# cs2mosa/Heterogeneous-MOE-for-Diffusion-models

Hardware: AMD Instinct MI355X
Metric: denoise-steps/sec (fwd+bwd) on 4x32x32 latents (higher is better)
Workload: dtype bf16

## Files before the change

### heterogeneous-moe-for-diffusion-models_amd/csrc/bwd6.hip

```cpp
#include "common.h"
#include "conv_args.h"
#include "conv6_common.h"
#include "hdmoe.h"
#include "conv6_body.h"
#include "conv7_body.h"
#include "wgrad6_body.h"
#include "wgrad7_body.h"
#include "wgrad8_body.h"
#include "conv6s_body.h"

namespace {

template <int MT, int NT, int TWS, int OT>
__global__ __launch_bounds__(512) void bwd6_kernel(C6Args c, W6Args a3, W6Args a5, int G6, int ibs, int obs) {
  const int b = blockIdx.x;
  if (b < G6) { conv6_body<MT, NT>(c, b, G6); return; }
  int r = b - G6;
  const int bx = r % ibs; r /= ibs;
  const int by = r % obs;
  const int z = r / obs;
  if (z < a3.chunks) wgrad6_body<3, TWS, OT, false>(a3, bx, by, z);
  else wgrad6_body<5, TWS, OT, false>(a5, bx, by, z - a3.chunks);
}

template <int MT, int NT, int TWS, int OT>
void launch_bwd6(const C6Plan& cp, const W6DualPlan& wp, hipStream_t stream) {
  static unsigned long long attr = 0;
  if (hdmoe_first_on_device(attr)) { (void)hipFuncSetAttribute((const void*)bwd6_kernel<MT, NT, TWS, OT>, hipFuncAttributeMaxDynamicSharedMemorySize, 160 * 1024); }
  const size_t lds = cp.lds > wp.lds ? cp.lds : wp.lds;
  const unsigned grid = cp.G + (unsigned)(wp.ibs * wp.obs * (wp.c[0].chunks + wp.c[1].chunks));
  hipLaunchKernelGGL((bwd6_kernel<MT, NT, TWS, OT>), dim3(grid), dim3(512), lds, stream, cp.a, wp.c[0], wp.c[1], (int)cp.G, wp.ibs, wp.obs);
}

template <int CO, int KMASK, int TWS, int OT, int EPI = 0>
__global__ __launch_bounds__(512) void bwd7_kernel(C7Args c, W6Args a3, W6Args a5, int G7, int ibs, int obs) {
  const int b = blockIdx.x;
  if (b < G7) { conv7_body<CO, KMASK, TWS == 4, EPI>(c, b, G7); return; }
  int r = b - G7;
  if (TWS == 5 && OT == 0) {
    const int nbx3 = a3.Cin / (32 * a3.icw), nby3 = a3.Cout / (32 * a3.ocw), n3 = nbx3 * nby3 * a3.chunks;
    if (r < n3) {
      const int bx = r % nbx3; r /= nbx3;
      const int by = r % nby3, z = r / nby3, pairs = a3.icw * a3.ocw;
      if (pairs == 0) wgrad7_body<3>(a3, bx, by, z);
      else if (pairs == 4) wgrad8_body3<4, 8>(a3, bx, by, z);
      else if (pairs == 2) wgrad8_body3<2, 8>(a3, bx, by, z);
      else wgrad8_body3<2, 16>(a3, bx, by, z);
      return;
    }
    r -= n3;
    const int bx = r % ibs; r /= ibs;
    wgrad7_body<5>(a5, bx, r % obs, r / obs);
  } else if (OT > 0) {
    const int bx = r % ibs; r /= ibs;
    const int by = r % obs;
    const int z = r / obs;
    if (z < a3.chunks) wgrad6_body<3, TWS, OT == 0 ? 1 : OT, false>(a3, bx, by, z);
    else wgrad6_body<5, TWS, OT == 0 ? 1 : OT, false>(a5, bx, by, z - a3.chunks);
  }
}

template <int CO, int KMASK, int TWS, int OT, int EPI = 0>
void launch_bwd7(const C7Plan& cp, const W6DualPlan& wp, hipStream_t stream) {
  static unsigned long long attr = 0;
  if (hdmoe_first_on_device(attr)) { (void)hipFuncSetAttribute((const void*)bwd7_kernel<CO, KMASK, TWS, OT, EPI>, hipFuncAttributeMaxDynamicSharedMemorySize, 160 * 1024); }
  const size_t clds = cp.lds + (EPI ? C7Lds<TWS == 4>::film_extra(CO) : 0);
  const size_t lds = clds > wp.lds ? clds : wp.lds;
  const int obs = OT == 0 ? wp.c[0].Cout / 32 : wp.obs;
  unsigned nw = (unsigned)(wp.ibs * obs * (wp.c[0].chunks + wp.c[1].chunks));
  if (OT == 0) nw = (unsigned)((wp.c[0].Cin / (32 * wp.c[0].icw)) * (wp.c[0].Cout / (32 * wp.c[0].ocw)) * wp.c[0].chunks + wp.ibs * obs * wp.c[1].chunks);
  hipLaunchKernelGGL((bwd7_kernel<CO, KMASK, TWS, OT, EPI>), dim3(cp.G + nw), dim3(512), lds, stream, cp.a, wp.c[0], wp.c[1], (int)cp.G, wp.ibs, obs);
}

template <int NT, int TWS, int OT>
__global__ __launch_bounds__(512) void bwd6s_kernel(C6SArgs c, W6Args a3, int G6, int ibs, int obs) {
  const int b = blockIdx.x;
  if (b < G6) { conv6s_body<NT>(c, b, G6); return; }
  int r = b - G6;
  const int bx = r % ibs; r /= ibs;
  wgrad6_body<3, TWS, OT, true>(a3, bx, r % obs, r / obs);
}
template <int NT, int TWS, int OT>
void launch_bwd6s(const C6SPlan& cp, const W6DualPlan& wp, hipStream_t stream) {
  static unsigned long long attr = 0;
  if (hdmoe_first_on_device(attr)) { (void)hipFuncSetAttribute((const void*)bwd6s_kernel<NT, TWS, OT>, hipFuncAttributeMaxDynamicSharedMemorySize, 160 * 1024); }
  const size_t lds = cp.lds > wp.lds ? cp.lds : wp.lds;
  const unsigned grid = cp.G + (unsigned)(wp.ibs * wp.obs * wp.c[0].chunks);
  hipLaunchKernelGGL((bwd6s_kernel<NT, TWS, OT>), dim3(grid), dim3(512), lds, stream, cp.sa, wp.c[0], (int)cp.G, wp.ibs, wp.obs);
}

}

extern "C" {

int hdmoe_conv_bwd6s(const void* x, const void* dy, const void* wd, void* dx, float* const* G, const int* seg, int ngroups, long wd_stride,
                     long wd_plane, int N, int H, int W, int Cin, int Cout, const int* kh, const int* kw, const int* pt, const int* pl,
                     float alpha, void* ws, long ws_bytes, const float* in_scale, const float* in_shift, int in_relu, int hi_only, hipStream_t stream) {
  if (!dx || !wd || ngroups < 1 || ngroups > HDMOE_MAX_GROUPS || Cout % 16) return 1;
  W6DualPlan wp;
  if (wgrad6_plan_split(x, dy, G, seg, ngroups, N, H, W, Cin, Cout, kh, kw, pt, pl, ws, ws_bytes, wp)) return 1;
  if ((in_scale == nullptr) != (in_shift == nullptr) || (in_scale && (ngroups != 1 || seg))) return HDMOE_EINVAL;
  wp.c[0].in_scale = in_scale; wp.c[0].in_shift = in_shift; wp.c[0].in_relu = in_relu;
  wp.c[0].hi_only = hi_only ? 1 : 0;
  const ConvArgs c = conv_dgrad_args(dy, wd, dx, seg, ngroups, wd_stride, N, H, W, Cin, Cout, kh, kw, pt, pl, alpha);
  C6SPlan cp;
  if (conv6s_plan(c, wd_plane, nullptr, cp)) return 1;
  cp.sa.nprod = hi_only ? 1 : 3;
  hdmoe_count_selection(HDMOE_SEL_BWD6S);
  conv_pick<2, 1>(cp.NT, [&](auto Nt) { conv_pick<5, 4>(wp.TWS, [&](auto Tws) { conv_pick<2, 1>(wp.OT, [&](auto Ot) {
    launch_bwd6s<decltype(Nt)::value, decltype(Tws)::value, decltype(Ot)::value>(cp, wp, stream);
  }); }); });
  return hdmoe_launch_status();
}

int hdmoe_conv_bwd6(const void* x, const void* dy, const void* wd, void* dx, float* const* G, const int* seg, int ngroups, long wd_stride,
                    int N, int H, int W, int Cin, int Cout, const int* kh, const int* kw, const int* pt, const int* pl, float alpha,
                    void* ws, long ws_bytes, int dtype, hipStream_t stream) {
  if (dtype != HDMOE_BF16 || !dx || !wd || ngroups < 1 || ngroups > HDMOE_MAX_GROUPS || Cout % 16) return 1;
  W6DualPlan wp;
  if (wgrad6_plan_dual(x, dy, G, seg, ngroups, N, H, W, Cin, Cout, kh, kw, pt, pl, ws, ws_bytes, dtype, wp)) return 1;
  const ConvArgs c = conv_dgrad_args(dy, wd, dx, seg, ngroups, wd_stride, N, H, W, Cin, Cout, kh, kw, pt, pl, alpha);
  {
    C7Plan cp7;
    if (!conv7_plan(c, dtype, cp7) && cp7.kmask == 3 && (cp7.w16 != 0) == (wp.TWS == 4)) {
      if (wp.TWS == 5) {
        hdmoe_count_selection(HDMOE_SEL_BWD7_32);
        if (wp.c[0].chunks) {
          hdmoe_count_selection(HDMOE_SEL_BWD7_32_WGRAD8);
          hdmoe_count_selection(wp.c[0].icw == 2 ? (wp.c[0].ocw == 2 ? HDMOE_SEL_WGRAD8_C22 : HDMOE_SEL_WGRAD8_C21)
                                                 : (wp.c[0].ocw == 2 ? HDMOE_SEL_WGRAD8_C12 : HDMOE_SEL_WGRAD8_C11));
        }
        if (wp.c[1].chunks) hdmoe_count_selection(HDMOE_SEL_BWD7_32_WGRAD7);
      } else {
        hdmoe_count_selection(wp.OT == 2 ? HDMOE_SEL_BWD7_16_OT2 : HDMOE_SEL_BWD7_16_OT1);
      }
      conv_pick<2, 1>(cp7.CO, [&](auto Co) {
        if (wp.TWS == 5) launch_bwd7<decltype(Co)::value, 3, 5, 0>(cp7, wp, stream);
        else conv_pick<2, 1>(wp.OT, [&](auto Ot) { launch_bwd7<decltype(Co)::value, 3, 4, decltype(Ot)::value>(cp7, wp, stream); });
      });
      return hdmoe_launch_status();
    }
  }
  C6Plan cp;
  if (conv6_plan(c, dtype, cp)) return 1;
  hdmoe_count_selection(HDMOE_SEL_BWD6);
  conv_pick<2, 1>(cp.MT, [&](auto M) { conv_pick<2, 1>(cp.NT, [&](auto Nt) { conv_pick<5, 4>(wp.TWS, [&](auto Tws) { conv_pick<2, 1>(wp.OT, [&](auto Ot) {
    launch_bwd6<decltype(M)::value, decltype(Nt)::value, decltype(Tws)::value, decltype(Ot)::value>(cp, wp, stream);
  }); }); }); });
  return hdmoe_launch_status();
}

int hdmoe_conv_bwd6_film(const void* x, const void* dy, const void* wd, void* dx, float* const* G, const int* seg, int ngroups, long wd_stride,
                         int N, int H, int W, int Cin, int Cout, const int* kh, const int* kw, const int* pt, const int* pl, float alpha,
                         void* ws, long ws_bytes, const void* film_u, const float* film_e, const unsigned char* film_mask, float* film_de,
                         float film_p, int dtype, hipStream_t stream) {
  if (dtype != HDMOE_BF16 || !dx || !wd || ngroups < 1 || ngroups > HDMOE_MAX_GROUPS || Cout % 16) return 1;
  if (!film_u || !film_e || !film_de || ((uintptr_t)film_u & 15) || ((uintptr_t)film_e & 15)) return 1;
  if (film_p < 0.f || film_p >= 1.f || (film_p > 0.f) != (film_mask != nullptr)) return HDMOE_EINVAL;
  W6DualPlan wp;
  if (wgrad6_plan_dual(x, dy, G, seg, ngroups, N, H, W, Cin, Cout, kh, kw, pt, pl, ws, ws_bytes, dtype, wp)) return 1;
  const ConvArgs c = conv_dgrad_args(dy, wd, dx, seg, ngroups, wd_stride, N, H, W, Cin, Cout, kh, kw, pt, pl, alpha);
  C7Plan cp7;
  if (conv7_plan(c, dtype, cp7) || cp7.kmask != 3 || (cp7.w16 != 0) != (wp.TWS == 4)) return 1;
  const bool big = wp.TWS == 5, small = wp.TWS == 4 && cp7.CO == 2 && wp.OT == 2;
  if (!big && !small) return 1;
  cp7.a.film_u = film_u; cp7.a.film_e = film_e; cp7.a.film_mask = film_mask; cp7.a.film_de = film_de;
  cp7.a.film_inv = film_p > 0.f ? 1.f / (1.f - film_p) : 1.f;
  hdmoe_count_selection(HDMOE_SEL_FILM_DGRAD);
  if (big) {
    hdmoe_count_selection(HDMOE_SEL_BWD7_32);
    if (wp.c[0].chunks) {
      hdmoe_count_selection(HDMOE_SEL_BWD7_32_WGRAD8);
      hdmoe_count_selection(wp.c[0].icw == 2 ? (wp.c[0].ocw == 2 ? HDMOE_SEL_WGRAD8_C22 : HDMOE_SEL_WGRAD8_C21)
                                             : (wp.c[0].ocw == 2 ? HDMOE_SEL_WGRAD8_C12 : HDMOE_SEL_WGRAD8_C11));
    }
    if (wp.c[1].chunks) hdmoe_count_selection(HDMOE_SEL_BWD7_32_WGRAD7);
    if (cp7.CO == 2) launch_bwd7<2, 3, 5, 0, 1>(cp7, wp, stream); else launch_bwd7<1, 3, 5, 0, 1>(cp7, wp, stream);
  } else {
    hdmoe_count_selection(HDMOE_SEL_BWD7_16_OT2);
    launch_bwd7<2, 3, 4, 2, 1>(cp7, wp, stream);
  }
  return hdmoe_launch_status();
}

}
```

### heterogeneous-moe-for-diffusion-models_amd/csrc/conv7.hip

```cpp
#include "conv_args.h"
#include "hdmoe.h"
#include "conv7_body.h"

namespace {

template <int CO, int KMASK, bool W16>
__global__ __launch_bounds__(512) void conv7_kernel(C7Args a) { conv7_body<CO, KMASK, W16>(a, blockIdx.x, gridDim.x); }

}

constexpr int C7_MIN_IMAGES = 192;

int conv7_plan(const ConvArgs& c, int dtype, C7Plan& plan) {
  if (dtype != HDMOE_BF16 || c.stride != 1 || c.ones || c.Cphys != c.Cin || c.Ipad != c.Cin || c.Cin % 32 || c.Cin > 256 || c.Cstore != c.Cout) return 1;
  if (c.Cout % 32 || c.Cout > 256) return 1;
  const bool w16 = c.H == 16;
  if (!((c.H == 32 && c.W == 32) || (c.H == 16 && c.W == 16)) || c.Ho != c.H || c.Wo != c.W || c.N < C7_MIN_IMAGES) return 1;
  int kmask = 0;
  long maxtaps = 0;
  for (int g = 0; g < c.ngroups; ++g) {
    const int k = c.kh[g];
    if (c.kw[g] != k || (k != 3 && k != 5 && k != 7) || c.pt[g] != (k - 1) / 2 || c.pl[g] != (k - 1) / 2) return 1;
    kmask |= k == 3 ? 1 : (k == 5 ? 2 : 4);
    if ((long)k * k > maxtaps) maxtaps = (long)k * k;
  }
  const long xbytes = (long)c.N * c.H * c.W * c.Cin * 2;
  const long wbytes = ((long)(c.ngroups - 1) * c.wstride + maxtaps * c.Cout * c.Cin) * 2;
  if (!conv_align_extent_ok({c.x, c.w, c.y, c.res}, {xbytes, wbytes, (long)c.N * c.H * c.W * c.Cout})) return 1;
  C7Args& a = plan.a;
  a.x = c.x; a.w = c.w; a.y = c.y; a.res = c.res; a.seg = c.seg; a.wstride = c.wstride;
  a.N = c.N; a.Cin = c.Cin; a.Cout = c.Cout; a.ngroups = c.ngroups; a.alpha = c.alpha; a.beta = c.beta;
  a.xbytes = (int)xbytes; a.wbytes = (int)wbytes;
  a.dbg = 0;
  a.film_u = nullptr; a.film_e = nullptr; a.film_mask = nullptr; a.film_de = nullptr; a.film_inv = 1.f;
  a.stamps = (unsigned long long*)hdmoe_debug_stamp_buffer();
  for (int g = 0; g < HDMOE_MAX_GROUPS; ++g) a.ks[g] = c.kh[g];
  conv_sort_groups_desc(a.ks, a.order, c.ngroups);
  const long gcap = 256;
  const long units = w16 ? (c.N + 1) / 2 + c.ngroups : c.N;
  plan.G = (unsigned)(units < gcap ? units : gcap);
  plan.CO = c.Cout % 64 == 0 ? 2 : 1;
  plan.w16 = w16 ? 1 : 0;
  plan.lds = w16 ? C7Lds<true>::BYTES : C7Lds<false>::BYTES;
  plan.kmask = (kmask & 4) ? 7 : 3;
  return 0;
}

template <int CO, int KMASK, bool W16>
static void conv7_launch_t(const C7Plan& p, hipStream_t stream) {
  static unsigned long long attr = 0;
  if (hdmoe_first_on_device(attr)) { (void)hipFuncSetAttribute((const void*)conv7_kernel<CO, KMASK, W16>, hipFuncAttributeMaxDynamicSharedMemorySize, C7Lds<W16>::BYTES); }
  hipLaunchKernelGGL((conv7_kernel<CO, KMASK, W16>), dim3(p.G), dim3(512), C7Lds<W16>::BYTES, stream, p.a);
}

void conv7_launch(const C7Plan& p, hipStream_t stream) {
  conv_pick<2, 1>(p.CO, [&](auto Co) { conv_pick<7, 3>(p.kmask, [&](auto Km) { conv_pick<1, 0>(p.w16 != 0, [&](auto W16) {
    conv7_launch_t<decltype(Co)::value, decltype(Km)::value, decltype(W16)::value != 0>(p, stream);
  }); }); });
}

int conv7_try_launch(const ConvArgs& c, int dtype, hipStream_t stream) {
  C7Plan plan;
  if (conv7_plan(c, dtype, plan)) return 1;
  hdmoe_count_selection(plan.w16 ? HDMOE_SEL_CONV7_16 : HDMOE_SEL_CONV7_32);
  conv7_launch(plan, stream);
  return hdmoe_launch_status();
}
```

### heterogeneous-moe-for-diffusion-models_amd/csrc/conv7_body.h

```cpp
#pragma once
#include <type_traits>
#include <utility>
#include "common.h"
#include "conv6_common.h"

namespace {

struct C7Args {
  const void* x; const void* w; void* y; const void* res; const int* seg;
  long wstride;
  int N, Cin, Cout, ngroups;
  int ks[HDMOE_MAX_GROUPS], order[HDMOE_MAX_GROUPS];
  float alpha, beta;
  int xbytes, wbytes;
  int dbg;
  unsigned long long* stamps;
  const void* film_u;
  const float* film_e;
  const unsigned char* film_mask;
  float* film_de;
  float film_inv;
};

template <bool W16> struct C7Geo;
template <> struct C7Geo<false> {
  static constexpr int IMG = 32, MB = 4, ROWB = 35 * 64, TILE = (32 * 35 + 3) * 64, WBUF = 8192, TCO = 4, PPW = 8, HBOFF = 0;
  static constexpr int ZBYTES = 38 * 64;
};
template <> struct C7Geo<true> {
  static constexpr int IMG = 16, MB = 2, ROWB = 19 * 64, TILE = (32 * 19 + 3) * 64, WBUF = 28672, TCO = 14, PPW = 4, HBOFF = 16 * 19 * 64;
  static constexpr int ZBYTES = HBOFF + 22 * 64;
};
template <bool W16> struct C7Lds {
  using GEO = C7Geo<W16>;
  static constexpr int T0 = 2 * GEO::WBUF;
  static constexpr int ZROW = T0 + 2 * GEO::TILE;
  static constexpr int BYTES = ZROW + GEO::ZBYTES;
  static constexpr int film_bytes(int co) { return 8 * (W16 ? 2 : 1) * 32 * co * 4; }
  static constexpr bool film_in_ring(int co) { return BYTES + film_bytes(co) > 160 * 1024; }
  static constexpr int film_extra(int co) { return film_in_ring(co) ? 0 : film_bytes(co); }
};

template <int KS, int CO, int TCO> struct C7Sched {
  static constexpr int T = TCO / CO;
  static constexpr int SPC = (KS + T - 1) / T;
  static constexpr int NS = KS * SPC;
  static constexpr int ky0(int i) { return (KS * i) / SPC; }
  static constexpr int nt(int i) { return (KS * (i + 1)) / SPC - (KS * i) / SPC; }
};

struct C7Unit { int g, n, n2, ks; };

template <typename F, int... I> DEVI void c7_static_for_impl(F&& f, std::integer_sequence<int, I...>) { (f(std::integral_constant<int, I>{}), ...); }
template <int N, typename F> DEVI void c7_static_for(F&& f) { c7_static_for_impl(f, std::make_integer_sequence<int, N>{}); }
template <int N> DEVI void c7_wait_barrier() { asm volatile("s_waitcnt vmcnt(%0) lgkmcnt(0)\n\ts_barrier" :: "n"(N) : "memory"); }

template <int CO, int KMASK, bool W16, int EPI = 0>
DEVI void conv7_body(const C7Args& a, const int bid, const int G) {
#if __HIP_DEVICE_COMPILE__
  using GEO = C7Geo<W16>;
  using L = C7Lds<W16>;
  constexpr int MB = GEO::MB, IMG = GEO::IMG, ROWB = GEO::ROWB, TILE = GEO::TILE, WBUF = GEO::WBUF, TCO = GEO::TCO, PPW = GEO::PPW;
  constexpr int T0 = L::T0, ZROW = L::ZROW;
  constexpr int NSTORE = MB * CO * 2;
  extern __shared__ __attribute__((aligned(1024))) unsigned char lds[];
  const int tid = threadIdx.x, lane = tid & 63;
  const int wave = __builtin_amdgcn_readfirstlane(tid >> 6);
  const int r = lane & 31, h = lane >> 5;
  const __amdgpu_buffer_rsrc_t rx = __builtin_amdgcn_make_buffer_rsrc(const_cast<void*>(a.x), 0, a.xbytes, 0x00020000);
  const __amdgpu_buffer_rsrc_t rw = __builtin_amdgcn_make_buffer_rsrc(const_cast<void*>(a.w), 0, a.wbytes, 0x00020000);
  const int CI = a.Cin >> 5;
  const int cin2 = a.Cin * 2;
  int nstamp = 0;
  auto stamp = [&](int tag) {
    if (a.stamps && bid == 0 && lane == 0 && nstamp < 63) {
      a.stamps[wave * 64 + nstamp] = ((unsigned long long)tag << 56) | (__builtin_amdgcn_s_memtime() & 0x00FFFFFFFFFFFFFFull);
      ++nstamp;
    }
  };
  stamp(1);

  int cum[HDMOE_MAX_GROUPS + 1];
  cum[0] = 0;
#pragma unroll
  for (int i = 0; i < HDMOE_MAX_GROUPS; ++i) {
    int cnt = 0;
    if (i < a.ngroups) { const int g = a.order[i]; cnt = a.seg ? a.seg[g + 1] - a.seg[g] : a.N; }
    cum[i + 1] = cum[i] + (W16 ? (cnt + 1) >> 1 : cnt);
  }
  const int total = cum[HDMOE_MAX_GROUPS];
  auto unit_at = [&](int q, C7Unit& u) -> bool {
    const int pos = q * G + ((q & 1) ? G - 1 - bid : bid);
    if (pos >= total) return false;
    int slot = 0;
#pragma unroll
    for (int i = 1; i < HDMOE_MAX_GROUPS; ++i) slot += (i < a.ngroups && pos >= cum[i]) ? 1 : 0;
    int base = 0, g = 0;
#pragma unroll
    for (int i = 0; i < HDMOE_MAX_GROUPS; ++i) if (i == slot) { base = cum[i]; g = a.order[i]; }
    int ks = 3;
#pragma unroll
    for (int i = 0; i < HDMOE_MAX_GROUPS; ++i) if (i == g) ks = a.ks[i];
    const int s0 = a.seg ? a.seg[g] : 0, s1 = a.seg ? a.seg[g + 1] : a.N;
    u.g = g; u.ks = ks;
    if (W16) { u.n = s0 + 2 * (pos - base); u.n2 = u.n + 1 < s1 ? u.n + 1 : -1; }
    else { u.n = s0 + pos - base; u.n2 = -1; }
    return true;
  };

  for (int i = tid; i < 33 * 12; i += 512) {
    const int off = (i / 12) * ROWB + (i % 12) * 16;
    *reinterpret_cast<uint4*>(lds + T0 + off) = make_uint4(0, 0, 0, 0);
    *reinterpret_cast<uint4*>(lds + T0 + TILE + off) = make_uint4(0, 0, 0, 0);
  }
  for (int i = tid; i < GEO::ZBYTES / 16; i += 512) *reinterpret_cast<uint4*>(lds + ZROW + i * 16) = make_uint4(0, 0, 0, 0);

  const int dpx = lane >> 2;
  const unsigned xlane = (unsigned)(dpx * cin2 + (((lane & 3) ^ (((3 + dpx) >> 2) & 3)) << 4));
  const unsigned wlane = (unsigned)(dpx * cin2 + (((lane & 3) ^ ((dpx >> 2) & 3)) << 4));
  int acol[7];
#pragma unroll
  for (int cc = 0; cc < 7; ++cc) {
    const int col = (W16 ? (r & 15) : r) + cc;
    acol[cc] = (col << 6) + ((h ^ ((col >> 2) & 3)) << 4) + (W16 ? (r >> 4) * GEO::HBOFF : 0);
  }
  const int wl = (r << 6) + ((h ^ ((r >> 2) & 3)) << 4);

  auto issue_tile = [&](const C7Unit& u, int c, int tb) {
    const int lbase = T0 + tb * TILE + 3 * 64;
#pragma unroll
    for (int k = 0; k < PPW; ++k) {
      if (W16) {
        const int img = k >> 1, row = 2 * wave + (k & 1);
        const int n = img ? u.n2 : u.n;
        const int so = (n * 16 + row) * 16 * cin2 + c * 64;
        const unsigned vo = n < 0 ? 0xFFFFFFFFu : xlane;
        __builtin_amdgcn_raw_ptr_buffer_load_lds(rx, (lptr_t)(lds + lbase + (img * 16 + row) * ROWB), 16, vo, n < 0 ? 0 : so, 0, 0);
      } else {
        const int row = 4 * wave + (k >> 1), half = k & 1;
        const int so = ((u.n * 32 + row) * 32 + half * 16) * cin2 + c * 64;
        __builtin_amdgcn_raw_ptr_buffer_load_lds(rx, (lptr_t)(lds + lbase + row * ROWB + half * 1024), 16, xlane, so, 0, 0);
      }
    }
  };
  auto issue_wstage = [&](int g, int ks, int c, int blk, int kx, int ky0, int nt, int sp) {
#pragma unroll
    for (int j = 0; j < (2 * TCO + 7) / 8; ++j) {
      const int pi = wave + 8 * j;
      const int ts = pi / (2 * CO), pc = pi % (2 * CO);
      if (ts < nt) {
        const int tap = (ky0 + ts) * ks + kx;
        const int so = (int)(((long)g * a.wstride + (long)(tap * a.Cout + blk * 32 * CO + pc * 16) * a.Cin) * 2) + c * 64;
        __builtin_amdgcn_raw_ptr_buffer_load_lds(rw, (lptr_t)(lds + sp * WBUF + pi * 1024), 16, wlane, so, 0, 0);
      }
    }
  };

  C7Unit cur, nxt;
  int q = 0;
  if (!unit_at(q, cur)) return;
  bool has_next = unit_at(q + 1, nxt);
  int tp = 0, sp = 0;
  auto nt0_of = [](int ks) { return ks == 3 ? C7Sched<3, CO, GEO::TCO>::nt(0) : (ks == 5 ? C7Sched<5, CO, GEO::TCO>::nt(0) : C7Sched<7, CO, GEO::TCO>::nt(0)); };
  const int nblk = a.Cout / (32 * CO);
  issue_wstage(cur.g, cur.ks, 0, 0, 0, 0, nt0_of(cur.ks), 0);
  issue_tile(cur, 0, 0);
  bool first = true;

  auto run_unit = [&](auto ks_tag) {
    constexpr int KS = decltype(ks_tag)::value;
    using S = C7Sched<KS, CO, TCO>;
    constexpr int P = (KS - 1) / 2, Q = 3 - P;
    for (int blk = 0; blk < nblk; ++blk) {
    const bool last_blk = blk == nblk - 1;
    f32x16 acc[MB][CO];
#pragma unroll
    for (int m = 0; m < MB; ++m)
#pragma unroll
      for (int b = 0; b < CO; ++b) acc[m][b] = (f32x16)(0.f);

    for (int c = 0; c < CI; ++c) {
      const bool last_chunk = c == CI - 1;
      const bool same_tile = last_chunk && !last_blk && CI == 1;
      const bool tile_next = (!last_chunk || (!last_blk && CI > 1) || (last_blk && has_next)) && !((a.dbg & 2) && last_chunk);
      const int tbase = T0 + tp * TILE;
      c7_static_for<S::NS>([&](auto s_c) {
        constexpr int s = decltype(s_c)::value;
        constexpr int kx = s / S::SPC, si = s % S::SPC;
        constexpr int ky0 = S::ky0(si), nt = S::nt(si);
        if (s == 0) {
          stamp(2);
          if (c == 0 && !first) c7_wait_barrier<NSTORE>();
          else c7_wait_barrier<0>();
          stamp(3);
        } else if (s == 1 && tile_next) {
          c7_wait_barrier<PPW>();
        } else {
          c7_wait_barrier<0>();
        }
        if (s + 1 < S::NS) {
          const int s1 = s + 1;
          issue_wstage(cur.g, KS, c, blk, s1 / S::SPC, S::ky0(s1 % S::SPC), S::nt(s1 % S::SPC), sp ^ 1);
        } else if (!last_chunk) {
          issue_wstage(cur.g, KS, c + 1, blk, 0, S::ky0(0), S::nt(0), sp ^ 1);
        } else if (!last_blk) {
          issue_wstage(cur.g, KS, 0, blk + 1, 0, S::ky0(0), S::nt(0), sp ^ 1);
        } else if (has_next) {
          issue_wstage(nxt.g, nxt.ks, 0, 0, 0, 0, nt0_of(nxt.ks), sp ^ 1);
        }
        if (s == 0 && tile_next) {
          if (!last_chunk) issue_tile(cur, c + 1, tp ^ 1); else if (!last_blk) issue_tile(cur, 0, tp ^ 1); else issue_tile(nxt, 0, tp ^ 1);
        }
        if (!(a.dbg & 1)) {
          const int wb = sp * WBUF;
          const int row0 = MB * (tid >> 6) - P + ky0;
#pragma unroll
          for (int k2 = 0; k2 < 2; ++k2) {
            bf16x8 xf[7 + MB - 1];
#pragma unroll
            for (int j = 0; j < nt + MB - 1; ++j) {
              const int row = row0 + j;
              const int sb = ((unsigned)row < (unsigned)IMG) ? tbase + row * ROWB : ZROW;
              xf[j] = *reinterpret_cast<const bf16x8*>(lds + ((acol[kx + Q] ^ (k2 << 5)) + sb));
            }
#pragma unroll
            for (int i = 0; i < nt; ++i) {
              bf16x8 wf[CO];
#pragma unroll
              for (int b = 0; b < CO; ++b)
                wf[b] = *reinterpret_cast<const bf16x8*>(lds + wb + (i * CO + b) * 2048 + (wl ^ (k2 << 5)));
#pragma unroll
              for (int m = 0; m < MB; ++m)
#pragma unroll
                for (int b = 0; b < CO; ++b)
                  acc[m][b] = __builtin_amdgcn_mfma_f32_32x32x16_bf16(wf[b], xf[m + i], acc[m][b], 0, 0, 0);
            }
          }
        }
        if ((CO == 1 || W16) && !(a.dbg & 16)) {
          constexpr int NRD = 2 * ((nt + MB - 1) + nt * CO), NMF = 2 * nt * MB * CO, LEAD = 4, R = NMF / NRD > 0 ? NMF / NRD : 1;
          __builtin_amdgcn_sched_group_barrier(0x100, LEAD < NRD ? LEAD : NRD, 0);
#pragma unroll
          for (int q = 0; q < NMF; ++q) {
            __builtin_amdgcn_sched_group_barrier(0x008, 1, 0);
            if ((q + 1) % R == 0 && LEAD + (q + 1) / R - 1 < NRD) __builtin_amdgcn_sched_group_barrier(0x100, 1, 0);
          }
        }
        sp ^= 1;
      });
      if (!same_tile) tp ^= 1;
    }
    const int cobase = blk * 32 * CO;
    stamp(4);
    if constexpr (EPI == 1) {
      constexpr int NIMG = W16 ? 2 : 1, NCH = 32 * CO;
      constexpr bool RING = L::film_in_ring(CO);
      static_assert(L::film_bytes(CO) <= WBUF, "the de partial sums do not fit a weight-ring buffer");
      bf16* Y = (bf16*)a.y;
      const bf16* U = (const bf16*)a.film_u;
      float* part = reinterpret_cast<float*>(lds + (RING ? (sp ^ 1) * WBUF : L::BYTES));
      if (RING) asm volatile("s_waitcnt lgkmcnt(0)\n\ts_barrier" ::: "memory");
      const int nimg = W16 ? ((r >> 4) ? cur.n2 : cur.n) : cur.n;
      const bool live = !W16 || nimg >= 0;
#pragma unroll
      for (int b = 0; b < CO; ++b)
#pragma unroll
        for (int p = 0; p < 2; ++p) {
          const int c0 = cobase + 32 * b + 16 * p + 8 * h;
          float ev[8], ds[8];
          {
            const float4 e0 = live ? *reinterpret_cast<const float4*>(a.film_e + (long)nimg * a.Cout + c0) : make_float4(0.f, 0.f, 0.f, 0.f);
            const float4 e1 = live ? *reinterpret_cast<const float4*>(a.film_e + (long)nimg * a.Cout + c0 + 4) : make_float4(0.f, 0.f, 0.f, 0.f);
            ev[0] = e0.x; ev[1] = e0.y; ev[2] = e0.z; ev[3] = e0.w; ev[4] = e1.x; ev[5] = e1.y; ev[6] = e1.z; ev[7] = e1.w;
          }
#pragma unroll
          for (int j = 0; j < 8; ++j) ds[j] = 0.f;
#pragma unroll
          for (int m = 0; m < MB; ++m) {
            const long o = (W16 ? (((long)nimg * 16 + 2 * wave + m) * 16 + (r & 15)) * a.Cout
                                : (((long)nimg * 32 + 4 * wave + m) * 32 + r) * a.Cout) + c0;
            float v[8];
#pragma unroll
            for (int e = 0; e < 8; ++e) v[e] = a.alpha * acc[m][b][8 * p + e];
            const C6Words pk = c6_pack_bf16(v);
            if (live) {
              const bf16x8 uu = *reinterpret_cast<const bf16x8*>(U + o);
              const unsigned mb = a.film_mask ? a.film_mask[o >> 3] : 0xFFu;
              bf16x8 out;
#pragma unroll
              for (int j = 0; j < 8; ++j) {
                const unsigned wj = pk.w[j >> 1];
                float g = __uint_as_float((j & 1) ? (wj & 0xFFFF0000u) : (wj << 16));
                const float uv = (float)uu[j];
                if (a.film_mask) g = (mb >> j) & 1u ? g * a.film_inv : 0.f;
                g *= mp_silu_grad_f(uv * ev[j]);
                ds[j] += g * uv;
                g *= ev[j];
                out[j] = (bf16)g;
              }
              *reinterpret_cast<bf16x8*>(Y + o) = out;
            }
          }
#pragma unroll
          for (int j = 0; j < 8; ++j) {
#pragma unroll
            for (int off = 1; off < (W16 ? 16 : 32); off <<= 1) ds[j] += __shfl_xor(ds[j], off);
          }
          if ((r & (W16 ? 15 : 31)) == 0) {
            float* dst = part + (wave * NIMG + (W16 ? (r >> 4) : 0)) * NCH + 32 * b + 16 * p + 8 * h;
            *reinterpret_cast<float4*>(dst) = make_float4(ds[0], ds[1], ds[2], ds[3]);
            *reinterpret_cast<float4*>(dst + 4) = make_float4(ds[4], ds[5], ds[6], ds[7]);
          }
        }
      asm volatile("s_waitcnt lgkmcnt(0)\n\ts_barrier" ::: "memory");
      if (tid < NIMG * NCH) {
        const int img = tid / NCH, c = tid % NCH;
        const int n = img ? cur.n2 : cur.n;
        float sum = 0.f;
#pragma unroll
        for (int w = 0; w < 8; ++w) sum += part[(w * NIMG + img) * NCH + c];
        if (n >= 0) a.film_de[(long)n * a.Cout + cobase + c] = sum;
      }
    } else if (!(a.dbg & 4)) {
      bf16* Y = (bf16*)a.y;
      const bf16* R = (const bf16*)a.res;
      const int nimg = W16 ? ((r >> 4) ? cur.n2 : cur.n) : cur.n;
      const bool live = !W16 || nimg >= 0;
#pragma unroll
      for (int m = 0; m < MB; ++m) {
        const long pix = W16 ? (((long)nimg * 16 + 2 * wave + m) * 16 + (r & 15)) * a.Cout
                             : (((long)nimg * 32 + 4 * wave + m) * 32 + r) * a.Cout;
#pragma unroll
        for (int b = 0; b < CO; ++b)
#pragma unroll
          for (int p = 0; p < 2; ++p) {
            float v[8];
#pragma unroll
            for (int e = 0; e < 8; ++e) v[e] = a.alpha * acc[m][b][8 * p + e];
            if (R && live) {
              const long o0 = pix + cobase + 32 * b + 16 * p + 4 * h;
              const bf16x4 r0 = *reinterpret_cast<const bf16x4*>(R + o0);
              const bf16x4 r1 = *reinterpret_cast<const bf16x4*>(R + o0 + 8);
#pragma unroll
              for (int e = 0; e < 4; ++e) { v[e] += a.beta * (float)r0[e]; v[4 + e] += a.beta * (float)r1[e]; }
            }
            const C6Words pk = c6_pack_bf16(v);
            if (live) *reinterpret_cast<uint4*>(Y + pix + cobase + 32 * b + 16 * p + 8 * h) = make_uint4(pk.w[0], pk.w[1], pk.w[2], pk.w[3]);
          }
      }
    } else {
#pragma unroll
      for (int m = 0; m < MB; ++m)
#pragma unroll
        for (int b = 0; b < CO; ++b) asm volatile("" :: "v"(acc[m][b]));
    }
    stamp(5);
    first = false;
    }
  };

  while (true) {
    if ((KMASK & 4) && cur.ks == 7) run_unit(std::integral_constant<int, 7>{});
    else if ((KMASK & 2) && cur.ks == 5) run_unit(std::integral_constant<int, 5>{});
    else run_unit(std::integral_constant<int, 3>{});
    first = false;
    if (!has_next) break;
    cur = nxt;
    ++q;
    has_next = unit_at(q + 1, nxt);
  }
#endif
}

}

struct ConvArgs;
struct C7Plan { C7Args a; unsigned G; int CO, kmask, w16; size_t lds; };
int conv7_plan(const ConvArgs& c, int dtype, C7Plan& plan);
void conv7_launch(const C7Plan& p, hipStream_t stream);
```

Measured before the change: 84.17.

## Precompute conv7 address strides and LDS group table, compile out debug stamps

Replaces the per-unit group lookup (prefix sums plus loops over groups) with a small LDS table that a ballot/readlane search reads. The host now precomputes 32-bit byte strides and packs each group's weight offset together with its kernel size, so the kernel updates tile and weight-stage offsets incrementally instead of doing 64-bit address arithmetic per load. Debug stamps and dbg flags become a compile-time DBG template parameter, selected only when stamps or dbg are set, so the normal kernel carries no timing code. Scheduling barriers are added around the MFMA section. Plans whose offsets would not fit in 32 bits fall back to another path.

Result: faster. 85.60, median of 6 (+1.7%).

```diff
diff --git a/heterogeneous-moe-for-diffusion-models_amd/csrc/bwd6.hip b/heterogeneous-moe-for-diffusion-models_amd/csrc/bwd6.hip
--- a/heterogeneous-moe-for-diffusion-models_amd/csrc/bwd6.hip
+++ b/heterogeneous-moe-for-diffusion-models_amd/csrc/bwd6.hip
@@ -32,10 +32,10 @@
   hipLaunchKernelGGL((bwd6_kernel<MT, NT, TWS, OT>), dim3(grid), dim3(512), lds, stream, cp.a, wp.c[0], wp.c[1], (int)cp.G, wp.ibs, wp.obs);
 }
 
-template <int CO, int KMASK, int TWS, int OT, int EPI = 0>
+template <int CO, int KMASK, int TWS, int OT, int EPI = 0, bool DBG = false>
 __global__ __launch_bounds__(512) void bwd7_kernel(C7Args c, W6Args a3, W6Args a5, int G7, int ibs, int obs) {
   const int b = blockIdx.x;
-  if (b < G7) { conv7_body<CO, KMASK, TWS == 4, EPI>(c, b, G7); return; }
+  if (b < G7) { conv7_body<CO, KMASK, TWS == 4, EPI, DBG>(c, b, G7); return; }
   int r = b - G7;
   if (TWS == 5 && OT == 0) {
     const int nbx3 = a3.Cin / (32 * a3.icw), nby3 = a3.Cout / (32 * a3.ocw), n3 = nbx3 * nby3 * a3.chunks;
@@ -60,16 +60,19 @@
   }
 }
 
-template <int CO, int KMASK, int TWS, int OT, int EPI = 0>
+template <int CO, int KMASK, int TWS, int OT, int EPI = 0, bool DBG = false>
 void launch_bwd7(const C7Plan& cp, const W6DualPlan& wp, hipStream_t stream) {
+  if constexpr (!DBG && EPI == 0 && (TWS == 5 || OT == 2)) {
+    if (cp.a.stamps || cp.a.dbg) { launch_bwd7<CO, KMASK, TWS, OT, 0, true>(cp, wp, stream); return; }
+  }
   static unsigned long long attr = 0;
-  if (hdmoe_first_on_device(attr)) { (void)hipFuncSetAttribute((const void*)bwd7_kernel<CO, KMASK, TWS, OT, EPI>, hipFuncAttributeMaxDynamicSharedMemorySize, 160 * 1024); }
+  if (hdmoe_first_on_device(attr)) { (void)hipFuncSetAttribute((const void*)bwd7_kernel<CO, KMASK, TWS, OT, EPI, DBG>, hipFuncAttributeMaxDynamicSharedMemorySize, 160 * 1024); }
   const size_t clds = cp.lds + (EPI ? C7Lds<TWS == 4>::film_extra(CO) : 0);
   const size_t lds = clds > wp.lds ? clds : wp.lds;
   const int obs = OT == 0 ? wp.c[0].Cout / 32 : wp.obs;
   unsigned nw = (unsigned)(wp.ibs * obs * (wp.c[0].chunks + wp.c[1].chunks));
   if (OT == 0) nw = (unsigned)((wp.c[0].Cin / (32 * wp.c[0].icw)) * (wp.c[0].Cout / (32 * wp.c[0].ocw)) * wp.c[0].chunks + wp.ibs * obs * wp.c[1].chunks);
-  hipLaunchKernelGGL((bwd7_kernel<CO, KMASK, TWS, OT, EPI>), dim3(cp.G + nw), dim3(512), lds, stream, cp.a, wp.c[0], wp.c[1], (int)cp.G, wp.ibs, obs);
+  hipLaunchKernelGGL((bwd7_kernel<CO, KMASK, TWS, OT, EPI, DBG>), dim3(cp.G + nw), dim3(512), lds, stream, cp.a, wp.c[0], wp.c[1], (int)cp.G, wp.ibs, obs);
 }
 
 template <int NT, int TWS, int OT>
diff --git a/heterogeneous-moe-for-diffusion-models_amd/csrc/conv7.hip b/heterogeneous-moe-for-diffusion-models_amd/csrc/conv7.hip
--- a/heterogeneous-moe-for-diffusion-models_amd/csrc/conv7.hip
+++ b/heterogeneous-moe-for-diffusion-models_amd/csrc/conv7.hip
@@ -4,8 +4,8 @@
 
 namespace {
 
-template <int CO, int KMASK, bool W16>
-__global__ __launch_bounds__(512) void conv7_kernel(C7Args a) { conv7_body<CO, KMASK, W16>(a, blockIdx.x, gridDim.x); }
+template <int CO, int KMASK, bool W16, bool DBG>
+__global__ __launch_bounds__(512) void conv7_kernel(C7Args a) { conv7_body<CO, KMASK, W16, 0, DBG>(a, blockIdx.x, gridDim.x); }
 
 }
 
@@ -27,35 +27,42 @@
   const long xbytes = (long)c.N * c.H * c.W * c.Cin * 2;
   const long wbytes = ((long)(c.ngroups - 1) * c.wstride + maxtaps * c.Cout * c.Cin) * 2;
   if (!conv_align_extent_ok({c.x, c.w, c.y, c.res}, {xbytes, wbytes, (long)c.N * c.H * c.W * c.Cout})) return 1;
+  const long gstride = c.wstride * 2, tapstride = (long)c.Cout * c.Cin * 2, imgstride = (long)c.H * c.W * c.Cin * 2;
+  if ((gstride & 7) || (c.ngroups - 1) * gstride + maxtaps * tapstride >= (1l << 31) || c.N * imgstride >= (1l << 31)) return 1;
   C7Args& a = plan.a;
-  a.x = c.x; a.w = c.w; a.y = c.y; a.res = c.res; a.seg = c.seg; a.wstride = c.wstride;
+  a.x = c.x; a.w = c.w; a.y = c.y; a.res = c.res; a.seg = c.seg;
   a.N = c.N; a.Cin = c.Cin; a.Cout = c.Cout; a.ngroups = c.ngroups; a.alpha = c.alpha; a.beta = c.beta;
   a.xbytes = (int)xbytes; a.wbytes = (int)wbytes;
   a.dbg = 0;
   a.film_u = nullptr; a.film_e = nullptr; a.film_mask = nullptr; a.film_de = nullptr; a.film_inv = 1.f;
   a.stamps = (unsigned long long*)hdmoe_debug_stamp_buffer();
-  for (int g = 0; g < HDMOE_MAX_GROUPS; ++g) a.ks[g] = c.kh[g];
-  conv_sort_groups_desc(a.ks, a.order, c.ngroups);
+  conv_sort_groups_desc(c.kh, a.order, c.ngroups);
+  for (int i = 0; i < HDMOE_MAX_GROUPS; ++i) a.gk[i] = (int)(a.order[i] * gstride) | c.kh[a.order[i]];
   const long gcap = 256;
   const long units = w16 ? (c.N + 1) / 2 + c.ngroups : c.N;
   plan.G = (unsigned)(units < gcap ? units : gcap);
   plan.CO = c.Cout % 64 == 0 ? 2 : 1;
+  a.tapstride = (int)tapstride; a.blkstride = 32 * plan.CO * c.Cin * 2;
+  a.imgstride = (int)imgstride; a.rowstride = c.W * c.Cin * 2;
   plan.w16 = w16 ? 1 : 0;
   plan.lds = w16 ? C7Lds<true>::BYTES : C7Lds<false>::BYTES;
   plan.kmask = (kmask & 4) ? 7 : 3;
   return 0;
 }
 
-template <int CO, int KMASK, bool W16>
+template <int CO, int KMASK, bool W16, bool DBG>
 static void conv7_launch_t(const C7Plan& p, hipStream_t stream) {
   static unsigned long long attr = 0;
-  if (hdmoe_first_on_device(attr)) { (void)hipFuncSetAttribute((const void*)conv7_kernel<CO, KMASK, W16>, hipFuncAttributeMaxDynamicSharedMemorySize, C7Lds<W16>::BYTES); }
-  hipLaunchKernelGGL((conv7_kernel<CO, KMASK, W16>), dim3(p.G), dim3(512), C7Lds<W16>::BYTES, stream, p.a);
+  if (hdmoe_first_on_device(attr)) { (void)hipFuncSetAttribute((const void*)conv7_kernel<CO, KMASK, W16, DBG>, hipFuncAttributeMaxDynamicSharedMemorySize, C7Lds<W16>::BYTES); }
+  hipLaunchKernelGGL((conv7_kernel<CO, KMASK, W16, DBG>), dim3(p.G), dim3(512), C7Lds<W16>::BYTES, stream, p.a);
 }
 
 void conv7_launch(const C7Plan& p, hipStream_t stream) {
   conv_pick<2, 1>(p.CO, [&](auto Co) { conv_pick<7, 3>(p.kmask, [&](auto Km) { conv_pick<1, 0>(p.w16 != 0, [&](auto W16) {
-    conv7_launch_t<decltype(Co)::value, decltype(Km)::value, decltype(W16)::value != 0>(p, stream);
+    if constexpr (decltype(Km)::value == 3) {
+      if (p.a.stamps || p.a.dbg) { conv7_launch_t<decltype(Co)::value, 3, decltype(W16)::value != 0, true>(p, stream); return; }
+    }
+    conv7_launch_t<decltype(Co)::value, decltype(Km)::value, decltype(W16)::value != 0, false>(p, stream);
   }); }); });
 }
 
diff --git a/heterogeneous-moe-for-diffusion-models_amd/csrc/conv7_body.h b/heterogeneous-moe-for-diffusion-models_amd/csrc/conv7_body.h
--- a/heterogeneous-moe-for-diffusion-models_amd/csrc/conv7_body.h
+++ b/heterogeneous-moe-for-diffusion-models_amd/csrc/conv7_body.h
@@ -8,9 +8,11 @@
 
 struct C7Args {
   const void* x; const void* w; void* y; const void* res; const int* seg;
-  long wstride;
   int N, Cin, Cout, ngroups;
-  int ks[HDMOE_MAX_GROUPS], order[HDMOE_MAX_GROUPS];
+  int order[HDMOE_MAX_GROUPS];
+  int gk[HDMOE_MAX_GROUPS];
+  int tapstride, blkstride;
+  int imgstride, rowstride;
   float alpha, beta;
   int xbytes, wbytes;
   int dbg;
@@ -35,7 +37,8 @@
   using GEO = C7Geo<W16>;
   static constexpr int T0 = 2 * GEO::WBUF;
   static constexpr int ZROW = T0 + 2 * GEO::TILE;
-  static constexpr int BYTES = ZROW + GEO::ZBYTES;
+  static constexpr int TAB = ZROW + GEO::ZBYTES;
+  static constexpr int BYTES = TAB + HDMOE_MAX_GROUPS * 16;
   static constexpr int film_bytes(int co) { return 8 * (W16 ? 2 : 1) * 32 * co * 4; }
   static constexpr bool film_in_ring(int co) { return BYTES + film_bytes(co) > 160 * 1024; }
   static constexpr int film_extra(int co) { return film_in_ring(co) ? 0 : film_bytes(co); }
@@ -49,19 +52,20 @@
   static constexpr int nt(int i) { return (KS * (i + 1)) / SPC - (KS * i) / SPC; }
 };
 
-struct C7Unit { int g, n, n2, ks; };
+struct C7Unit { int n, n2, gk, xb, wrow; };
 
 template <typename F, int... I> DEVI void c7_static_for_impl(F&& f, std::integer_sequence<int, I...>) { (f(std::integral_constant<int, I>{}), ...); }
 template <int N, typename F> DEVI void c7_static_for(F&& f) { c7_static_for_impl(f, std::make_integer_sequence<int, N>{}); }
 template <int N> DEVI void c7_wait_barrier() { asm volatile("s_waitcnt vmcnt(%0) lgkmcnt(0)\n\ts_barrier" :: "n"(N) : "memory"); }
 
-template <int CO, int KMASK, bool W16, int EPI = 0>
+template <int CO, int KMASK, bool W16, int EPI = 0, bool DBG = false>
 DEVI void conv7_body(const C7Args& a, const int bid, const int G) {
 #if __HIP_DEVICE_COMPILE__
   using GEO = C7Geo<W16>;
   using L = C7Lds<W16>;
   constexpr int MB = GEO::MB, IMG = GEO::IMG, ROWB = GEO::ROWB, TILE = GEO::TILE, WBUF = GEO::WBUF, TCO = GEO::TCO, PPW = GEO::PPW;
-  constexpr int T0 = L::T0, ZROW = L::ZROW;
+  constexpr int T0 = L::T0, ZROW = L::ZROW, TAB = L::TAB;
+  constexpr int NWJ = (2 * TCO + 7) / 8;
   constexpr int NSTORE = MB * CO * 2;
   extern __shared__ __attribute__((aligned(1024))) unsigned char lds[];
   const int tid = threadIdx.x, lane = tid & 63;
@@ -71,40 +75,43 @@
   const __amdgpu_buffer_rsrc_t rw = __builtin_amdgcn_make_buffer_rsrc(const_cast<void*>(a.w), 0, a.wbytes, 0x00020000);
   const int CI = a.Cin >> 5;
   const int cin2 = a.Cin * 2;
+  const int dbg = DBG ? a.dbg : 0;
   int nstamp = 0;
-  auto stamp = [&](int tag) {
-    if (a.stamps && bid == 0 && lane == 0 && nstamp < 63) {
-      a.stamps[wave * 64 + nstamp] = ((unsigned long long)tag << 56) | (__builtin_amdgcn_s_memtime() & 0x00FFFFFFFFFFFFFFull);
-      ++nstamp;
-    }
-  };
+  unsigned t_iss = 0;
+  auto ticks = [&]() -> unsigned { if constexpr (DBG) return (unsigned)__builtin_amdgcn_s_memtime(); else return 0u; };
+  auto stampv = [&](int tag, unsigned long long v) {
+    if constexpr (DBG) {
+      if (a.stamps && bid == 0 && lane == 0 && nstamp < 63) { a.stamps[wave * 64 + nstamp] = ((unsigned long long)tag << 56) | v; ++nstamp; }
+    }
+  };
+  auto stamp = [&](int tag) { if constexpr (DBG) stampv(tag, __builtin_amdgcn_s_memtime() & 0x00FFFFFFFFFFFFFFull); };
   stamp(1);
 
-  int cum[HDMOE_MAX_GROUPS + 1];
-  cum[0] = 0;
-#pragma unroll
-  for (int i = 0; i < HDMOE_MAX_GROUPS; ++i) {
-    int cnt = 0;
-    if (i < a.ngroups) { const int g = a.order[i]; cnt = a.seg ? a.seg[g + 1] - a.seg[g] : a.N; }
-    cum[i + 1] = cum[i] + (W16 ? (cnt + 1) >> 1 : cnt);
+  int total = 0;
+  {
+    int e0 = 0x7FFFFFFF, e1 = 0, e2 = 0, e3 = 0;
+#pragma unroll
+    for (int i = 0; i < HDMOE_MAX_GROUPS; ++i) {
+      if (i < a.ngroups) {
+        const int g = a.order[i];
+        const int s0 = a.seg ? a.seg[g] : 0, s1 = a.seg ? a.seg[g + 1] : a.N;
+        if (lane == i) { e0 = total; e1 = s0; e2 = s1; e3 = a.gk[i]; }
+        total += W16 ? (s1 - s0 + 1) >> 1 : s1 - s0;
+      }
+    }
+    if (lane < HDMOE_MAX_GROUPS) *reinterpret_cast<int4*>(lds + TAB + lane * 16) = make_int4(e0, e1, e2, e3);
   }
-  const int total = cum[HDMOE_MAX_GROUPS];
   auto unit_at = [&](int q, C7Unit& u) -> bool {
     const int pos = q * G + ((q & 1) ? G - 1 - bid : bid);
     if (pos >= total) return false;
-    int slot = 0;
-#pragma unroll
-    for (int i = 1; i < HDMOE_MAX_GROUPS; ++i) slot += (i < a.ngroups && pos >= cum[i]) ? 1 : 0;
-    int base = 0, g = 0;
-#pragma unroll
-    for (int i = 0; i < HDMOE_MAX_GROUPS; ++i) if (i == slot) { base = cum[i]; g = a.order[i]; }
-    int ks = 3;
-#pragma unroll
-    for (int i = 0; i < HDMOE_MAX_GROUPS; ++i) if (i == g) ks = a.ks[i];
-    const int s0 = a.seg ? a.seg[g] : 0, s1 = a.seg ? a.seg[g + 1] : a.N;
-    u.g = g; u.ks = ks;
+    const int4 e = *reinterpret_cast<const int4*>(lds + TAB + (lane & (HDMOE_MAX_GROUPS - 1)) * 16);
+    const int slot = __builtin_popcountll(__ballot(e.x <= pos) & ((1ull << HDMOE_MAX_GROUPS) - 1)) - 1;
+    const int base = __builtin_amdgcn_readlane(e.x, slot), s0 = __builtin_amdgcn_readlane(e.y, slot), s1 = __builtin_amdgcn_readlane(e.z, slot);
+    u.gk = __builtin_amdgcn_readlane(e.w, slot);
     if (W16) { u.n = s0 + 2 * (pos - base); u.n2 = u.n + 1 < s1 ? u.n + 1 : -1; }
     else { u.n = s0 + pos - base; u.n2 = -1; }
+    u.xb = u.n * a.imgstride;
+    u.wrow = (u.gk & 7) * a.tapstride;
     return true;
   };
 
@@ -116,8 +123,12 @@
   for (int i = tid; i < GEO::ZBYTES / 16; i += 512) *reinterpret_cast<uint4*>(lds + ZROW + i * 16) = make_uint4(0, 0, 0, 0);
 
   const int dpx = lane >> 2;
-  const unsigned xlane = (unsigned)(dpx * cin2 + (((lane & 3) ^ (((3 + dpx) >> 2) & 3)) << 4));
+  const unsigned xlane = (unsigned)((tid >> 6) * MB * a.rowstride + dpx * cin2 + (((lane & 3) ^ (((3 + dpx) >> 2) & 3)) << 4));
   const unsigned wlane = (unsigned)(dpx * cin2 + (((lane & 3) ^ ((dpx >> 2) & 3)) << 4));
+  auto wvoff = [&](int j, int wrow) -> unsigned {
+    const int pi = (tid >> 6) + 8 * j;
+    return wlane + (unsigned)((pi / (2 * CO)) * wrow + (pi % (2 * CO)) * (16 * cin2));
+  };
   int acol[7];
 #pragma unroll
   for (int cc = 0; cc < 7; ++cc) {
@@ -126,44 +137,45 @@
   }
   const int wl = (r << 6) + ((h ^ ((r >> 2) & 3)) << 4);
 
-  auto issue_tile = [&](const C7Unit& u, int c, int tb) {
-    const int lbase = T0 + tb * TILE + 3 * 64;
+  auto issue_tile = [&](const C7Unit& u, int coff, int tb) {
+    const int lw = T0 + 3 * 64 + (tb ? TILE : 0) + wave * (MB * ROWB);
+    int so = u.xb + coff;
 #pragma unroll
     for (int k = 0; k < PPW; ++k) {
       if (W16) {
-        const int img = k >> 1, row = 2 * wave + (k & 1);
-        const int n = img ? u.n2 : u.n;
-        const int so = (n * 16 + row) * 16 * cin2 + c * 64;
-        const unsigned vo = n < 0 ? 0xFFFFFFFFu : xlane;
-        __builtin_amdgcn_raw_ptr_buffer_load_lds(rx, (lptr_t)(lds + lbase + (img * 16 + row) * ROWB), 16, vo, n < 0 ? 0 : so, 0, 0);
+        const int img = k >> 1;
+        const bool absent = img && u.n2 < 0;
+        __builtin_amdgcn_raw_ptr_buffer_load_lds(rx, (lptr_t)(lds + lw + (img * 16 + (k & 1)) * ROWB), 16, absent ? 0xFFFFFFFFu : xlane, absent ? 0 : so, 0, 0);
+        so += (k & 1) ? a.imgstride - a.rowstride : a.rowstride;
       } else {
-        const int row = 4 * wave + (k >> 1), half = k & 1;
-        const int so = ((u.n * 32 + row) * 32 + half * 16) * cin2 + c * 64;
-        __builtin_amdgcn_raw_ptr_buffer_load_lds(rx, (lptr_t)(lds + lbase + row * ROWB + half * 1024), 16, xlane, so, 0, 0);
+        __builtin_amdgcn_raw_ptr_buffer_load_lds(rx, (lptr_t)(lds + lw + (k >> 1) * ROWB + (k & 1) * 1024), 16, xlane, so, 0, 0);
+        so += a.rowstride >> 1;
       }
     }
   };
-  auto issue_wstage = [&](int g, int ks, int c, int blk, int kx, int ky0, int nt, int sp) {
-#pragma unroll
-    for (int j = 0; j < (2 * TCO + 7) / 8; ++j) {
+  auto issue_wstage = [&](int so, const unsigned (&wv)[NWJ], int nt, int sp) {
+#pragma unroll
+    for (int j = 0; j < NWJ; ++j) {
       const int pi = wave + 8 * j;
-      const int ts = pi / (2 * CO), pc = pi % (2 * CO);
-      if (ts < nt) {
-        const int tap = (ky0 + ts) * ks + kx;
-        const int so = (int)(((long)g * a.wstride + (long)(tap * a.Cout + blk * 32 * CO + pc * 16) * a.Cin) * 2) + c * 64;
-        __builtin_amdgcn_raw_ptr_buffer_load_lds(rw, (lptr_t)(lds + sp * WBUF + pi * 1024), 16, wlane, so, 0, 0);
-      }
+      if (pi < nt * 2 * CO) __builtin_amdgcn_raw_ptr_buffer_load_lds(rw, (lptr_t)(lds + (sp ? WBUF : 0) + pi * 1024), 16, wv[j], so, 0, 0);
     }
   };
 
   C7Unit cur, nxt;
   int q = 0;
   if (!unit_at(q, cur)) return;
+  unsigned td0 = ticks();
   bool has_next = unit_at(q + 1, nxt);
+  stampv(11, ticks() - td0);
   int tp = 0, sp = 0;
   auto nt0_of = [](int ks) { return ks == 3 ? C7Sched<3, CO, GEO::TCO>::nt(0) : (ks == 5 ? C7Sched<5, CO, GEO::TCO>::nt(0) : C7Sched<7, CO, GEO::TCO>::nt(0)); };
   const int nblk = a.Cout / (32 * CO);
-  issue_wstage(cur.g, cur.ks, 0, 0, 0, 0, nt0_of(cur.ks), 0);
+  {
+    unsigned wv[NWJ];
+#pragma unroll
+    for (int j = 0; j < NWJ; ++j) wv[j] = wvoff(j, cur.wrow);
+    issue_wstage(cur.gk & ~7, wv, nt0_of(cur.gk & 7), 0);
+  }
   issue_tile(cur, 0, 0);
   bool first = true;
 
@@ -171,6 +183,10 @@
     constexpr int KS = decltype(ks_tag)::value;
     using S = C7Sched<KS, CO, TCO>;
     constexpr int P = (KS - 1) / 2, Q = 3 - P;
+    unsigned wv[NWJ];
+#pragma unroll
+    for (int j = 0; j < NWJ; ++j) wv[j] = wvoff(j, cur.wrow);
+    int wblk = cur.gk & ~7;
     for (int blk = 0; blk < nblk; ++blk) {
     const bool last_blk = blk == nblk - 1;
     f32x16 acc[MB][CO];
@@ -182,8 +198,10 @@
     for (int c = 0; c < CI; ++c) {
       const bool last_chunk = c == CI - 1;
       const bool same_tile = last_chunk && !last_blk && CI == 1;
-      const bool tile_next = (!last_chunk || (!last_blk && CI > 1) || (last_blk && has_next)) && !((a.dbg & 2) && last_chunk);
-      const int tbase = T0 + tp * TILE;
+      const bool tile_next = (!last_chunk || (!last_blk && CI > 1) || (last_blk && has_next)) && !((dbg & 2) && last_chunk);
+      const int tbase = T0 + (tp ? TILE : 0);
+      const int wchunk = wblk + c * 64;
+      int wcol = wchunk;
       c7_static_for<S::NS>([&](auto s_c) {
         constexpr int s = decltype(s_c)::value;
         constexpr int kx = s / S::SPC, si = s % S::SPC;
@@ -198,21 +216,28 @@
         } else {
           c7_wait_barrier<0>();
         }
+        const unsigned ti0 = ticks();
         if (s + 1 < S::NS) {
-          const int s1 = s + 1;
-          issue_wstage(cur.g, KS, c, blk, s1 / S::SPC, S::ky0(s1 % S::SPC), S::nt(s1 % S::SPC), sp ^ 1);
+          constexpr int s1 = s + 1, k1 = S::ky0(s1 % S::SPC);
+          if (s1 % S::SPC == 0) { wcol += a.tapstride; asm volatile("" : "+s"(wcol)); }
+          issue_wstage(wcol + k1 * cur.wrow, wv, S::nt(s1 % S::SPC), sp ^ 1);
         } else if (!last_chunk) {
-          issue_wstage(cur.g, KS, c + 1, blk, 0, S::ky0(0), S::nt(0), sp ^ 1);
+          issue_wstage(wchunk + 64, wv, S::nt(0), sp ^ 1);
         } else if (!last_blk) {
-          issue_wstage(cur.g, KS, 0, blk + 1, 0, S::ky0(0), S::nt(0), sp ^ 1);
+          issue_wstage(wblk + a.blkstride, wv, S::nt(0), sp ^ 1);
         } else if (has_next) {
-          issue_wstage(nxt.g, nxt.ks, 0, 0, 0, 0, nt0_of(nxt.ks), sp ^ 1);
+          unsigned wn[NWJ];
+#pragma unroll
+          for (int j = 0; j < NWJ; ++j) wn[j] = wvoff(j, nxt.wrow);
+          issue_wstage(nxt.gk & ~7, wn, nt0_of(nxt.gk & 7), sp ^ 1);
         }
         if (s == 0 && tile_next) {
-          if (!last_chunk) issue_tile(cur, c + 1, tp ^ 1); else if (!last_blk) issue_tile(cur, 0, tp ^ 1); else issue_tile(nxt, 0, tp ^ 1);
-        }
-        if (!(a.dbg & 1)) {
-          const int wb = sp * WBUF;
+          if (!last_chunk) issue_tile(cur, (c + 1) * 64, tp ^ 1); else if (!last_blk) issue_tile(cur, 0, tp ^ 1); else issue_tile(nxt, 0, tp ^ 1);
+        }
+        if constexpr (DBG) t_iss += ticks() - ti0;
+        __builtin_amdgcn_sched_barrier(0);
+        if (!(dbg & 1)) {
+          const int wb = sp ? WBUF : 0;
           const int row0 = MB * (tid >> 6) - P + ky0;
 #pragma unroll
           for (int k2 = 0; k2 < 2; ++k2) {
@@ -237,7 +262,8 @@
             }
           }
         }
-        if ((CO == 1 || W16) && !(a.dbg & 16)) {
+        __builtin_amdgcn_sched_barrier(0);
+        if ((CO == 1 || W16) && !(dbg & 16)) {
           constexpr int NRD = 2 * ((nt + MB - 1) + nt * CO), NMF = 2 * nt * MB * CO, LEAD = 4, R = NMF / NRD > 0 ? NMF / NRD : 1;
           __builtin_amdgcn_sched_group_barrier(0x100, LEAD < NRD ? LEAD : NRD, 0);
 #pragma unroll
@@ -251,7 +277,9 @@
       if (!same_tile) tp ^= 1;
     }
     const int cobase = blk * 32 * CO;
+    wblk += a.blkstride;
     stamp(4);
+    stampv(10, t_iss); t_iss = 0;
     if constexpr (EPI == 1) {
       constexpr int NIMG = W16 ? 2 : 1, NCH = 32 * CO;
       constexpr bool RING = L::film_in_ring(CO);
@@ -321,7 +349,7 @@
         for (int w = 0; w < 8; ++w) sum += part[(w * NIMG + img) * NCH + c];
         if (n >= 0) a.film_de[(long)n * a.Cout + cobase + c] = sum;
       }
-    } else if (!(a.dbg & 4)) {
+    } else if (!(dbg & 4)) {
       bf16* Y = (bf16*)a.y;
       const bf16* R = (const bf16*)a.res;
       const int nimg = W16 ? ((r >> 4) ? cur.n2 : cur.n) : cur.n;
@@ -360,14 +388,16 @@
   };
 
   while (true) {
-    if ((KMASK & 4) && cur.ks == 7) run_unit(std::integral_constant<int, 7>{});
-    else if ((KMASK & 2) && cur.ks == 5) run_unit(std::integral_constant<int, 5>{});
+    if ((KMASK & 4) && (cur.gk & 7) == 7) run_unit(std::integral_constant<int, 7>{});
+    else if ((KMASK & 2) && (cur.gk & 7) == 5) run_unit(std::integral_constant<int, 5>{});
     else run_unit(std::integral_constant<int, 3>{});
     first = false;
     if (!has_next) break;
     cur = nxt;
     ++q;
+    td0 = ticks();
     has_next = unit_at(q + 1, nxt);
+    stampv(11, ticks() - td0);
   }
 #endif
 }
```
